# fdeguire03/InteriorPoint-GPU

Hardware: AMD Instinct MI355X
Metric: Newton iters/sec, dense QP n=8192, 1/2/4/8 GPUs; achieved % fp64 roofline (higher is better)
Workload: dtype f64

## Files before the change

### interiorpoint-gpu_amd/csrc/ipm_blas.hip

```cpp
#include <atomic>
#include "ipm_common.h"
#include <cstdio>
#include "ipm_mfma.h"

#include <algorithm>
#include <map>
#include <mutex>
#include <queue>
#include <cmath>
#include <tuple>
#include <vector>
#include <cstdlib>
#include <cstring>

namespace ipm {

static inline int64_t cdiv(int64_t a, int64_t b) { return (a + b - 1) / b; }

template <bool VEC>
__device__ __forceinline__ void gemv_row(int64_t row, int64_t cols, double alpha, const double* __restrict__ M,
                                         int64_t ldm, const double* __restrict__ x, double beta,
                                         double* __restrict__ y) {
  const int lane = threadIdx.x & 63;
  const double* mr = M + row * ldm;
// ... 1197 lines not shown
      if (16 * jt >= next_nb) break;
      const int64_t col0 = k0 + nb + 16 * jt;
      dbl4 acc;
#pragma unroll
      for (int r = 0; r < 4; ++r)
        acc[r] = (rfold && 16 * jt + fk + 4 * r < next_nb)
                     ? (FUSED ? ld_sc1(&A[(col0 + fk + 4 * r) * lda + row]) : A[(col0 + fk + 4 * r) * lda + row])
                     : 0.0;
      const double* sb = stage + jl * SLAB + fk * 16 + fr;
#pragma unroll
      for (int P = 0; P < 8; ++P)
#pragma unroll
        for (int s4 = 0; s4 < 4; ++s4)
          acc = __builtin_amdgcn_mfma_f64_16x16x4f64(-sb[(16 * P + 4 * s4) * 16], x[P][s4], acc, 0, 0, 0);
      if (rfold) {
#pragma unroll
        for (int r = 0; r < 4; ++r)
          if (16 * jt + fk + 4 * r < next_nb) {
            if (FUSED) st_sc1(&A[(col0 + fk + 4 * r) * lda + row], acc[r]);
            else A[(col0 + fk + 4 * r) * lda + row] = acc[r];
          }
      }
    }
  }
  }
  }
  if (done) {
    asm volatile("s_waitcnt vmcnt(0)" ::: "memory");
    __syncthreads();
    if (tid == 0) __hip_atomic_store(done, 1u, __ATOMIC_RELAXED, __HIP_MEMORY_SCOPE_AGENT);
  }
}

struct BlockArgs {
  int64_t n = 0, lda = 0;
  double* A = nullptr;
  int* info = nullptr;
  double* wsA = nullptr;
  double* wsB = nullptr;
  unsigned* ctl = nullptr;
  const unsigned* prevfail = nullptr;
  int64_t cb = 0;
  int wa = 0, wbw = 0;
  int nla = 0, nra = 0, nrb = 0, la_tj = 0, nlab = 0;
  int64_t ns = 0;
  int nnf = 0;
  GemmArgs la32, la, la128, s;
  int nla32 = 0, la32_T = 0, nla64 = 0, nla128 = 0;
  int trace = 0;
  int64_t rag_r0 = 0;
  int rag_n = 0, nrag = 0;
  int64_t s_full = 0;
  double* sscr = nullptr;
  unsigned* sflag = nullptr;
  int64_t nstrip = 0, f0 = 0;
  GemmArgs s2;
  int rag_K = CH_NB;
  int64_t rag_cp = 0;
  int ntail = 0, tail_r = 0, tail_R = 0, tail_K = 0;
  int64_t tail_o = 0, tail_k0 = 0;
};
__device__ __forceinline__ unsigned cu_key() {
  const unsigned hw = __builtin_amdgcn_s_getreg((31 << 11) | 4);
  const unsigned xcc = __builtin_amdgcn_s_getreg((31 << 11) | 20);
  return ((xcc & 15u) << 8) | ((hw >> 8) & 0xFFu);
}
// ... 12 lines not shown
  __syncthreads();
}

#ifdef IPM_ROLE_TRACE
__device__ unsigned long long ipm_role_trace[8192 * 4];
struct RoleTrace {
  bool on;
  int ticket;
  unsigned long long t0;
  int role = -1;
  unsigned long long wake = 0, loaded = 0;
  __device__ RoleTrace(bool o, int t) : on(o && t < 8192), ticket(t), t0(__builtin_amdgcn_s_memrealtime()) {}
  __device__ ~RoleTrace() {
    if (on && threadIdx.x == 0) {
      const unsigned lo = wake ? (unsigned)(loaded - t0) : (unsigned)ticket;
      ipm_role_trace[4 * ticket] = (unsigned long long)lo | ((unsigned long long)(unsigned)role << 32);
      ipm_role_trace[4 * ticket + 1] = t0;
      ipm_role_trace[4 * ticket + 2] = __builtin_amdgcn_s_memrealtime();
      ipm_role_trace[4 * ticket + 3] = wake ? wake : cu_key();
    }
  }
};
#define ROLE(r) (rt.role = (r))
#define ROLE_STAMP(f) (rt.f = __builtin_amdgcn_s_memrealtime())
__device__ unsigned long long ipm_fold_trace[32 * 12];
#define FOLD_SLOT ((frole == 0 ? 0 : 16) + ftile)
#define FOLD_STAMP(i) do { if (rt.on && ftile < 16 && tid == 0) ipm_fold_trace[FOLD_SLOT * 12 + (i)] = __builtin_amdgcn_s_memrealtime(); } while (0)
#else
#define FOLD_STAMP(i) do {} while (0)
#define ROLE(r) ((void)0)
#define ROLE_STAMP(f) ((void)0)
#endif

template <bool VEC, bool FASTS, int LAZY>
__device__ __forceinline__ void potrf_block_body(const BlockArgs& b, int64_t t, BlockSmem& sm, int& sflag) {
  const int tid = threadIdx.x;
  unsigned* const failw = &b.ctl[CTL_FAIL];
#ifdef IPM_ROLE_TRACE
  RoleTrace rt(b.trace != 0, (int)t);
#endif
  const int64_t t_launch = t;
  auto prev_failed = [&]() {
    const unsigned pf = ld_ctl(const_cast<unsigned*>(b.prevfail));
    if (pf == 0) return false;
    if (t_launch == 0 && tid == 0) __hip_atomic_store(&b.ctl[CTL_FAIL], pf, __ATOMIC_RELAXED, __HIP_MEMORY_SCOPE_AGENT);
    return true;
  };
  if (!(VEC && t < b.nla32 && (b.la32.K % 128) == 0) && prev_failed()) return;
  unsigned* la_done = b.ctl + CTL_HDR;
  unsigned* pa_done = la_done + (b.n + 63) / 64;
  int64_t fo = 0, fsrc = 0;
  int fni = 0, fnj = 0, fnp = 0;
  int ftile = 0, frole = 9;
  unsigned* fdone = nullptr;
  bool fwait = false;
  const bool la_fold = VEC && t < b.nla32 && (b.la32.K % 128) == 0;
  if (t < b.nla && !la_fold) {
    ROLE(0);
    int64_t rb;
    if (t < b.nla32) {
      mfma_tile<32, false, VEC, 2, true>(b.la32, t, sm.g32);
      int64_t i = (int64_t)((sqrt(8.0 * (double)t + 1.0) - 1.0) * 0.5);
      while ((i + 1) * (i + 2) / 2 <= t) ++i;
      while (i * (i + 1) / 2 > t) --i;
      rb = i >> 1;
    } else if (t - b.nla32 < b.nla64) {
      const int64_t t64 = t - b.nla32;
// ... 251 lines not shown
      const bool live = p < R * r && j <= i;
      double acc = 0.0;
      if (live)
        for (int k = q; k < K; k += 16) acc = fma(Ls[i * K + k], Ls[j * K + k], acc);
#pragma unroll
      for (int m = 8; m >= 1; m >>= 1) acc += __shfl_xor(acc, m, 16);
      if (live && q == 0) Cs[i * r + j] = ld_sc1(&b.A[(o + j) * lda + o + i]) - acc;
    }
    __syncthreads();
    int fcol = 0;
    for (int j = 0; j < r; ++j) {
      if (tid >= j && tid < R) {
        double v = Cs[tid * r + j];
        for (int k = 0; k < j; ++k) v = fma(-Cs[tid * r + k], Cs[j * r + k], v);
        Ts[tid] = v;
      }
      __syncthreads();
      const double piv = Ts[j], dv = rsqrt_pivot(piv);
      if (!(piv > 0.0) && fcol == 0) fcol = j + 1;
      if (tid >= j && tid < R) Cs[tid * r + j] = tid == j ? piv * dv : Ts[tid] * dv;
      __syncthreads();
    }
    if (tid < R)
      for (int j = 0; j < r && j <= tid; ++j) b.A[(o + j) * lda + o + tid] = Cs[tid * r + j];
    if (fcol && tid == 0) {
      atomicCAS(b.info, 0, (int)(o + fcol));
      __hip_atomic_store(failw, (unsigned)(o + fcol), __ATOMIC_RELAXED, __HIP_MEMORY_SCOPE_AGENT);
    }
    return;
  }
  if (kind == K_RAG) {
    ROLE(12);
    const int64_t o = b.cb + b.wa + b.wbw, cp = b.rag_cp;
    const int64_t m = b.n - o, r0 = b.rag_r0;
    const int rn = b.rag_n, KR = b.rag_K;
    double* xr = sm.d.sD;
    for (int e = tid; e < rn * KR; e += 256) {
      const int q = e / KR, k = e - q * KR;
      xr[e] = b.A[(cp + k) * b.lda + o + r0 + q];
    }
    __syncthreads();
    const int64_t j = t * 256 + tid;
    if (j < m) {
      double* cj = b.A + (o + j) * b.lda + o + r0;
      double acc[8];
#pragma unroll
      for (int q = 0; q < 8; ++q) acc[q] = (q < rn && j <= r0 + q) ? cj[q] : 0.0;
      const double* xp = b.A + cp * b.lda + o + j;
#pragma unroll 16
      for (int k = 0; k < KR; ++k) {
        const double xj = xp[k * b.lda];
#pragma unroll
        for (int q = 0; q < 8; ++q)
          if (q < rn) acc[q] = fma(-xj, xr[q * KR + k], acc[q]);
      }
#pragma unroll
      for (int q = 0; q < 8; ++q)
        if (q < rn && j <= r0 + q) cj[q] = acc[q];
    }
    return;
  }
  if (kind == K_TILE) {
    ROLE(4);
    {
        const int64_t st0 = t;
        const bool strip = st0 < b.nstrip;
        const int64_t st = strip ? st0 : st0 - b.nstrip, u = strip ? -1 : st - b.s_full;
        const int sp = u < 0 ? 0 : ((u & 1) ? 2 : 1);
        const int64_t p = u < 0 ? 0 : (u >> 1);
        GemmArgs g = b.s;
        if (strip) {
          g.ni = b.s2.ni;
          g.nj = b.s2.nj;
          g.X = b.s2.X;
          g.Y = b.s2.Y;
          g.C = b.s2.C;
          g.rowmajor = 1;
          g.xcd_remap = 0;
          g.tiles_i = b.s2.tiles_i;
          g.tiles_j = b.s2.tiles_j;
          g.nblk = b.s2.nblk;
        }
        mfma_tile<128, false, VEC, 2, false, false, (FASTS && VEC) ? 1 : 0, (FASTS && VEC) ? LAZY : 0>(
            g, strip ? st + (st >= 1 ? 1 : 0)
                     : b.f0 + (u < 0 ? st : b.s_full + p),
            sm.g128, sp, b.sscr + p * (128 * 128), b.sflag + p, -1, -1, b.info, failw);
    }
  }
}

template <bool VEC, bool FASTS = false, int LAZY = 0>
__global__ __launch_bounds__(256, 2) void k_potrf_block(BlockArgs b_arg) {
  IPM_KARGS(BlockArgs, b, b_arg);
  __shared__ BlockSmem sm;
  __shared__ int sticket, sflag;
  if (threadIdx.x == 0) sticket = (int)atomicAdd(&b.ctl[CTL_TICKET], 1u);
  __syncthreads();
  potrf_block_body<VEC, FASTS, LAZY>(b, __builtin_amdgcn_readfirstlane(sticket), sm, sflag);
}

static constexpr int64_t PANEL_WS = PF_DINV + 36 * 256;

__global__ void k_zero2(unsigned* a, int64_t na, unsigned* b, int64_t nb) {
  const int64_t i = (int64_t)blockIdx.x * 256 + threadIdx.x;
  if (i < na) a[i] = 0u;
  else if (i - na < nb) b[i - na] = 0u;
}
__global__ void k_zero2_border(unsigned* a, int64_t na, unsigned* b, int64_t nb, BorderJob j) {
  const int64_t i = (int64_t)blockIdx.x * 256 + threadIdx.x;
  if (i < na) a[i] = 0u;
  else if (i - na < nb) b[i - na] = 0u;
  else {
    const int64_t c = i - na - nb;
    if (c < j.N) j.H[c * j.ldh + j.N] = j.scale * j.g[c];
    else if (c == j.N) j.H[j.N * j.ldh + j.N] = j.corner;
  }
}
static void zero2(hipStream_t st, void* a, int64_t na, void* b, int64_t nb) {
  const int64_t tot = na + nb;
  if (tot > 0)
    hipLaunchKernelGGL(k_zero2, dim3((unsigned)cdiv(tot, 256)), dim3(256), 0, st, reinterpret_cast<unsigned*>(a), na,
                       reinterpret_cast<unsigned*>(b), nb);
}

static int num_cus();
static double split_makespan(int slots, const std::vector<std::pair<int64_t, double>>& items) {
  std::priority_queue<double, std::vector<double>, std::greater<double>> q;
  for (int i = 0; i < slots; ++i) q.push(0.0);
  double mk = 0.0;
  for (const auto& it : items)
    for (int64_t k = 0; k < it.first; ++k) {
      const double t = q.top() + it.second;
      q.pop();
      q.push(t);
      mk = std::max(mk, t);
    }
  return mk;
}
static std::vector<std::pair<int64_t, double>> launch_items(int64_t nla, int64_t nchd, int64_t nnf, bool pb,
                                                            int64_t nrag, int64_t nstrip, int64_t ns, int64_t q,
                                                            double tc, double lac, int64_t nra, int64_t nrb,
                                                            int64_t sa, int64_t sb) {
  std::vector<std::pair<int64_t, double>> it = {{nla, lac}, {1, 0.6}, {nchd, 0.66}, {nnf, 0.8}, {pb ? 1 : 0, 1.25},
                                                {nrag, 0.1 * tc}};
  const int64_t e1 = nstrip + ns - q, e2 = e1 + 2 * q;
  auto span = [&](int64_t a, int64_t z) {
    const int64_t w1 = std::max<int64_t>(0, std::min(z, e1) - a);
    const int64_t w2 = std::max<int64_t>(0, std::min(z, e2) - std::max(a, e1));
    if (w1 > 0) it.push_back({w1, tc});
    if (w2 > 0) it.push_back({w2, 0.55 * tc});
  };
  sa = std::min(sa, e2);
  sb = std::min(std::max(sb, sa), e2);
  span(0, sa);
  it.push_back({nra, 0.5});
  span(sa, sb);
  it.push_back({nrb, 0.5});
  span(sb, e2);
  return it;
}
static int64_t plan_split(int64_t nla, int64_t nchd, int64_t nnf, bool pb, int64_t nrag, int64_t ns, int64_t nrows,
                          int64_t cap, double tc = 1.0, int64_t nstrip = 0, double lac = 0.8, int64_t nra = -1,
                          int64_t sa = -1, int64_t sb = -1) {
  if (ns < 64) return 0;
  const int slots = 2 * num_cus();
  if (nra < 0) {
    nra = nrows;
    sa = sb = nstrip + ns;
  }
  const int64_t nrb = nrows - nra;
  auto mk = [&](int64_t q) {
    int64_t a = sa, z = sb;
    return split_makespan(slots, launch_items(nla, nchd, nnf, pb, nrag, nstrip, ns, q, tc, lac, nra, nrb, a, z));
  };
  const double m0 = mk(0);
  double best = m0;
  int64_t bq = 0;
  for (int64_t q = 8; q <= std::min(ns, cap); q += 8) {
    const double m = mk(q);
    if (m < best - 0.02) { best = m; bq = q; }
  }
  return bq;
}

struct PairPlan {
  std::vector<int> kind;
  std::vector<int64_t> f1;
};
static PairPlan potrf_pair_plan(int64_t n, int64_t ncols, int64_t nblocks) {
  PairPlan pl;
  pl.kind.assign(nblocks, 0);
  pl.f1.assign(nblocks, 0);
  static const bool on = [] { const char* e = getenv("IPM_PAIR"); return !(e && e[0] == '0'); }();
  static const int64_t minrows = [] { const char* e = getenv("IPM_PAIR_MIN"); return e ? atoll(e) : 6144LL; }();
  if (!on || ncols < n - 8) return pl;
  int64_t last = -1;
  for (int64_t e = 2; e + 1 < nblocks; e += 2) {
    if (n - (e + 2) * CH_NB < minrows) break;
    last = e;
  }
  if (last < 0) return pl;
  pl.kind[1] = 1;
  for (int64_t e = 2; e <= last; e += 2) {
    pl.kind[e] = 2;
    if (e < last) pl.kind[e + 1] = 1;
  }
  return pl;
}

static unsigned long long wall_ticks(unsigned us) {
  static long long khz = -1;
  if (khz < 0) {
    int dev = 0, v = 0;
    hipGetDevice(&dev);
    khz = (hipDeviceGetAttribute(&v, hipDeviceAttributeWallClockRate, dev) == hipSuccess && v > 0) ? v : 100000;
  }
  const unsigned long long t = (unsigned long long)us * (unsigned long long)khz / 1000ull;
  return t > 0 ? t : 1;
}
constexpr unsigned SPIN_US_DEFAULT = 1000000;
static void set_spin_ticks(int which, unsigned us) {
  const unsigned long long t = wall_ticks(us ? us : SPIN_US_DEFAULT);
  int cur = 0, cnt = 0;
  hipGetDevice(&cur);
  if (hipGetDeviceCount(&cnt) != hipSuccess || cnt < 1) cnt = 1;
  for (int d = 0; d < cnt; ++d) {
    if (hipSetDevice(d) != hipSuccess) continue;
    hipMemcpyToSymbol(HIP_SYMBOL(ipm_spin_ticks), &t, sizeof(t), which * sizeof(t), hipMemcpyHostToDevice);
  }
  hipSetDevice(cur);
}
void set_potrf_spin_limit_us(unsigned us) { set_spin_ticks(0, us); }

struct BlockLaunch {
  BlockArgs b;
  int64_t grid = 0;
  int inst = 4;
};
static void potrf_plan(int64_t n, double* A, int64_t lda, int* info, double* ws, int64_t ncols,
                       std::vector<BlockLaunch>& out) {
  out.clear();
  const int64_t nblocks = cdiv(ncols, CH_NB), cw = block_ctl_words(n);
  unsigned* ctl0 = reinterpret_cast<unsigned*>(ws + 2 * PANEL_WS);
  const bool vec = ((lda & 1) == 0) && ((((uintptr_t)A) & 15) == 0);
  const char* erag = getenv("IPM_RAG");
  const bool rag_on = erag ? erag[0] != '0' : n > 5120;
  const char* esp = getenv("IPM_SPLIT");
  const bool split_on = !(esp && esp[0] == '0');
  const char* elz = getenv("IPM_LAZYC");
  const bool lazy_on = !(elz && elz[0] == '0');
  const bool lazy2_on = lazy_on && !(elz && elz[0] == '1');
  PairPlan pl = potrf_pair_plan(n, ncols, nblocks);
  const char* etl = getenv("IPM_TAIL");
  const bool tail_on = !(etl && etl[0] == '0');
  int64_t nemit = nblocks;
  int tail_r = 0;
  if (tail_on && nblocks >= 2 && pl.kind[nblocks - 2] == 0) {
    const int64_t cbl = (nblocks - 1) * CH_NB;
    if (ncols - cbl <= 8 && n - cbl <= 16) {
      nemit = nblocks - 1;
      tail_r = (int)(ncols - cbl);
    }
  }
  for (int64_t bk = 0; bk < nemit; ++bk) {
    const int kind = pl.kind[bk];
    const int64_t Kla = kind == 2 ? 2 * CH_NB : CH_NB;
    BlockArgs b;
    b.n = n;
    b.lda = lda;
    b.A = A;
    b.info = info;
    b.wsA = ws;
    b.wsB = ws + PANEL_WS;
    b.ctl = ctl0 + 8 + bk * cw;
    b.prevfail = bk == 0 ? ctl0 : ctl0 + 8 + (bk - 1) * cw + CTL_FAIL;
    const int64_t cb = bk * CH_NB, wb = std::min<int64_t>(CH_NB, ncols - cb);
    b.cb = cb;
    b.wa = (int)std::min<int64_t>(wb, PF_NB);
    b.wbw = (int)(wb - b.wa);
    if (bk > 0) {
      const int64_t cp = cb - Kla;
      const int64_t ni = n - cb;
      GemmArgs& c = b.la32;
      c.ni = std::min<int64_t>(ni, 128);
// ... 44 lines not shown
      b.nla = b.nla32 + b.nla64 + b.nla128;
      b.la_tj = (int)a.tiles_j;
      b.nlab = (int)cdiv(ni, 64);
      const int64_t m = n - cb - wb;
      b.rag_cp = cb - CH_NB;
      b.rag_K = CH_NB;
      if (m > 0 && kind == 1) {
        if (bk >= 1 && pl.kind[bk - 1] == 2) {
          const int64_t me = m + CH_NB;
          const int64_t rn = (rag_on && me > 128 && (me & 127) != 0 && (me & 127) <= 8) ? (me & 127) : 0;
          const int64_t mF = m - rn;
          GemmArgs& g = b.s;
          g.ni = g.nj = mF;
          g.K = 2 * CH_NB;
          g.X = g.Y = A + (cb - 3 * CH_NB) * lda + cb + wb;
          g.ldx = g.ldy = lda;
          g.C = A + (cb + wb) * lda + cb + wb;
          g.ldc = lda;
          g.sub = 1;
          g.tri = 1;
          g.xcd_remap = 1;
          g.tiles_i = cdiv(mF, 128);
          g.nblk = g.tiles_i * (g.tiles_i + 1) / 2;
          b.f0 = pl.f1[bk - 1];
          b.s_full = g.nblk - b.f0;
          b.ns = b.s_full;
        }
      } else if (m > 0 && kind == 2) {
        int64_t ms = m;
        if (rag_on && m > 128 && (m & 127) != 0 && (m & 127) <= 8) {
          ms = m - (m & 127);
          b.rag_r0 = ms;
          b.rag_n = (int)(m & 127);
          b.nrag = (int)cdiv(m, 256);
          b.rag_cp = cp;
          b.rag_K = (int)Kla;
        }
        const int64_t o = cb + wb, mF = ms - CH_NB;
        GemmArgs& s2 = b.s2;
        s2.ni = ms;
        s2.nj = CH_NB;
        s2.K = Kla;
        s2.X = s2.Y = A + cp * lda + o;
        s2.ldx = s2.ldy = lda;
        s2.C = A + o * lda + o;
        s2.ldc = lda;
        s2.sub = 1;
        s2.tri = 1;
        s2.rowmajor = 1;
        s2.xcd_remap = 0;
        s2.tiles_i = cdiv(ms, 128);
        s2.tiles_j = 2;
        s2.nblk = s2.tiles_i * 2;
        b.nstrip = s2.nblk - 1;
        GemmArgs& g = b.s;
        g = s2;
        g.rowmajor = 0;
        g.ni = g.nj = mF;
        g.X = g.Y = A + cp * lda + o + CH_NB;
        g.C = A + (o + CH_NB) * lda + o + CH_NB;
        g.xcd_remap = 1;
        g.tiles_i = cdiv(mF, 128);
        g.tiles_j = 0;
        g.nblk = g.tiles_i * (g.tiles_i + 1) / 2;
        const bool last = bk + 1 >= nblocks || pl.kind[bk + 1] != 1;
        const int64_t f1 = last ? g.nblk : std::max<int64_t>(0, std::min<int64_t>(g.nblk, (g.nblk - b.nstrip) / 2));
        pl.f1[bk] = f1;
        b.f0 = 0;
        b.s_full = f1;
        b.ns = b.nstrip + f1;
      } else if (m > 0) {
        GemmArgs& g = b.s;
        int64_t ms = m;
        if (rag_on && m > 128 && (m & 127) != 0 && (m & 127) <= 8) {
          ms = m - (m & 127);
          b.rag_r0 = ms;
          b.rag_n = (int)(m & 127);
          b.nrag = (int)cdiv(m, 256);
        }
        g.ni = g.nj = ms;
        g.K = CH_NB;
        g.X = g.Y = A + cp * lda + cb + wb;
        g.ldx = g.ldy = lda;
        g.C = A + (cb + wb) * lda + cb + wb;
        g.ldc = lda;
        g.sub = 1;
        g.tri = 1;
        g.xcd_remap = 1;
        g.tiles_i = cdiv(ms, 128);
        g.nblk = g.tiles_i * (g.tiles_i + 1) / 2;
        b.ns = g.nblk;
        b.s_full = b.ns;
      }
    }
    if (tail_r > 0 && bk == nemit - 1) {
      b.ns = b.s_full = b.nstrip = 0;
      b.nrag = 0;
      b.ntail = 1;
      b.tail_r = tail_r;
      b.tail_o = cb + CH_NB;
      b.tail_R = (int)(n - b.tail_o);
      b.tail_k0 = bk > 0 ? cb - CH_NB : 0;
      b.tail_K = (int)(b.tail_o - b.tail_k0);
    }
#ifdef IPM_ROLE_TRACE
    {
      static const int tb = [] { const char* e = getenv("IPM_TRACE_BLOCK"); return e ? atoi(e) : -1; }();
      b.trace = bk == tb;
    }
#endif
    b.nra = (int)cdiv(std::max<int64_t>(n - cb - b.wa, 0), PF_RB);
// ... 9 lines not shown
    if (b.s_full > 0 && split_here) {
      static std::mutex mu;
      static std::map<std::tuple<int64_t, int64_t, int>, std::vector<int64_t>> cache;
      const int nchd_h = b.wbw > 0 ? (b.wbw + PF_RB - 1) / PF_RB : 0;
      const double tc = b.s.K > CH_NB ? 1.6 : 1.0, lac = Kla > CH_NB ? 1.6 : 0.8;
      const int64_t nra_h = b.nra - nchd_h;
      int64_t q = 0;
      {
        std::lock_guard<std::mutex> lk(mu);
        auto& v = cache[{n, ncols, (lazy_on ? 4 : 0) | (lazy2_on ? 8 : 0) | (vec ? 16 : 0)}];
        if ((int64_t)v.size() < nblocks) v.assign(nblocks, -1);
        if (v[bk] < 0) {
          v[bk] = plan_split(b.nla, nchd_h, b.nnf, b.wbw > 0, b.nrag, b.s_full, nra_h + b.nrb, potrf_split_cap(n),
                             tc, b.nstrip, lac);
          static const bool dbg = getenv("IPM_SPLIT_DEBUG") != nullptr;
          if (dbg)
            fprintf(stderr, "potrf n=%ld block %ld: %ld trailing tiles, split %ld\n", (long)n, (long)bk, (long)b.ns,
                    (long)v[bk]);
        }
        q = v[bk];
      }
      b.s_full -= q;
      b.ns = b.nstrip + b.s_full + 2 * q;
      b.sscr = ws + potrf_split_scratch_off(n);
      b.sflag = b.ctl + block_ctl_words(n) - potrf_split_cap(n);
    }
    BlockLaunch L;
    L.grid = b.nla + 1 + b.nra + b.nnf + (b.wbw > 0 ? 1 + b.nrb : 0) + b.nrag + b.ns + b.ntail;
    const bool fasts = fasts_on && b.ns > 0 && (b.s.ni % 128) == 0 && (b.s.K % 32) == 0;
    const bool lazy = lazy_on && fasts && b.s.K == CH_NB && b.nstrip == 0 && b.s_full == b.ns;
    const bool lazy2 = lazy2_on && fasts && b.s.K == 2 * CH_NB && b.nstrip + b.s_full == b.ns &&
                       (b.nstrip == 0 || b.s2.K == 2 * CH_NB) && (b.nrag == 0 || b.rag_K <= 2 * CH_NB);
    L.inst = (vec && lazy) ? 0 : (vec && lazy2) ? 1 : (vec && fasts) ? 2 : vec ? 3 : 4;
    L.b = b;
    out.push_back(L);
  }
}

static void launch_block(hipStream_t st, const BlockLaunch& L) {
  const dim3 g((unsigned)L.grid), t(256);
  switch (L.inst) {
    case 0: hipLaunchKernelGGL((k_potrf_block<true, true, 1>), g, t, 0, st, L.b); break;
    case 1: hipLaunchKernelGGL((k_potrf_block<true, true, 2>), g, t, 0, st, L.b); break;
    case 2: hipLaunchKernelGGL((k_potrf_block<true, true>), g, t, 0, st, L.b); break;
    case 3: hipLaunchKernelGGL((k_potrf_block<true, false>), g, t, 0, st, L.b); break;
    default: hipLaunchKernelGGL((k_potrf_block<false, false>), g, t, 0, st, L.b); break;
  }
}

void potrf_lower_fused(hipStream_t st, int64_t n, double* A, int64_t lda, int* info, double* ws, int64_t ncols,
                       const BorderJob* border) {
  if (ncols < 0 || ncols > n) ncols = n;
  if (border && ncols <= 0) border_rhs(st, border->N, border->H, border->ldh, border->g, border->scale);
  if (ncols <= 0) {
    hipMemsetAsync(info, 0, sizeof(int), st);
    return;
  }
  thread_local std::vector<BlockLaunch> plan;
  potrf_plan(n, A, lda, info, ws, ncols, plan);
  unsigned* ctl0 = reinterpret_cast<unsigned*>(ws + 2 * PANEL_WS);
  if (border) {
    const int64_t nz = 8 + (int64_t)plan.size() * block_ctl_words(n), tot = 1 + nz + border->N + 1;
    hipLaunchKernelGGL(k_zero2_border, dim3((unsigned)cdiv(tot, 256)), dim3(256), 0, st, reinterpret_cast<unsigned*>(info),
                       (int64_t)1, ctl0, nz, *border);
  } else {
    zero2(st, info, 1, ctl0, 8 + (int64_t)plan.size() * block_ctl_words(n));
  }
  for (const BlockLaunch& L : plan) launch_block(st, L);
}

static int num_cus() {
  static int ncu = -1;
  if (ncu < 0) {
    int dev = 0, v = 0;
    hipGetDevice(&dev);
    ncu = (hipDeviceGetAttribute(&v, hipDeviceAttributeMultiprocessorCount, dev) == hipSuccess && v > 0) ? v : 256;
  }
  return ncu;
// ... 831 lines not shown
```

### interiorpoint-gpu_amd/csrc/ipm_mfma.h

```cpp
#pragma once
#include <algorithm>
#include <map>
#include <mutex>
#include <queue>
#include <tuple>
#include <type_traits>
#include <vector>

#include "ipm_common.h"

namespace ipm {

#ifdef IPM_TILE_STAMPS
__device__ unsigned long long ipm_tile_stamps[4096 * 8];
#define IPM_TSTAMP(k) do { if (threadIdx.x == 0 && blockIdx.x < 4096) ipm_tile_stamps[blockIdx.x * 8 + (k)] = __builtin_amdgcn_s_memtime(); } while (0)
#define IPM_TSTAMPR(k) do { if (threadIdx.x == 0 && blockIdx.x < 4096) ipm_tile_stamps[blockIdx.x * 8 + (k)] = __builtin_amdgcn_s_memrealtime(); } while (0)
#else
#define IPM_TSTAMP(k) do {} while (0)
#define IPM_TSTAMPR(k) do {} while (0)
#endif

struct GemmArgs {
  int64_t ni = 0, nj = 0, K = 0;
  const double* X = nullptr;
// ... 26 lines not shown
      reinterpret_cast<unsigned long long*>(const_cast<double*>(p)), __ATOMIC_RELAXED, __HIP_MEMORY_SCOPE_AGENT));
}
__device__ __forceinline__ void st_sc1(double* p, double v) {
  __hip_atomic_store(reinterpret_cast<unsigned long long*>(p), (unsigned long long)__double_as_longlong(v),
                     __ATOMIC_RELAXED, __HIP_MEMORY_SCOPE_AGENT);
}

static __device__ unsigned long long ipm_spin_ticks[2] = {100000000ull, 100000000ull};
__device__ __forceinline__ void spin_fail(int* info, unsigned* failw) {
  if (info) atomicCAS(info, 0, POTRF_INFO_SPIN);
  __threadfence();
  if (failw) atomicCAS(failw, 0u, 0xFFFFFFF0u);
}
template <int SLEEP, int WHICH = 0, class Done>
__device__ __forceinline__ bool spin_until(int* info, unsigned* failw, Done done) {
  if (done()) return true;
  unsigned long long t0 = 0;
  for (unsigned it = 0;; ++it) {
    __builtin_amdgcn_s_sleep(SLEEP);
    if (done()) return true;
    if ((it & 15u) != 0u) continue;
    const unsigned long long now = __builtin_amdgcn_s_memrealtime();
    if (it == 0) {
      t0 = now;
      continue;
    }
    if (failw && __hip_atomic_load(failw, __ATOMIC_RELAXED, __HIP_MEMORY_SCOPE_AGENT) != 0u) return false;
    if (now - t0 > ipm_spin_ticks[WHICH]) {
      spin_fail(info, failw);
      return false;
    }
  }
}

template <int BM_, int WJ = 2>
struct MfCfg {
  static constexpr int BM = BM_, BK = 16, NT = 128 * WJ;
  static constexpr int LD = BM + 16;
  static constexpr int PT = BK * BM / NT;
  static constexpr int TPR = BM / PT;
  static constexpr int TWI = BM / 32;
  static constexpr int TWJ = BM / (16 * WJ);
};

template <int BM_, int WJ = 2>
struct alignas(16) MfSmem {
  alignas(16) double sX[2][MfCfg<BM_, WJ>::BK * MfCfg<BM_, WJ>::LD];
  alignas(16) double sY[2][MfCfg<BM_, WJ>::BK * MfCfg<BM_, WJ>::LD];
};

template <int BM_, bool WEIGHT, bool VEC, int WJ = 2, bool SC1OUT = false, bool SPLITADD = false, int LOOP = 0,
          int LAZYC = 0, bool CST = false>
__device__ __forceinline__ void mfma_tile(const GemmArgs& a, int64_t Lw, MfSmem<BM_, WJ>& sm, int SPLIT = 0,
                                          double* part = nullptr, unsigned* pflag = nullptr, int64_t kb = -1,
                                          int64_t ke = -1, int* sinfo = nullptr, unsigned* failw = nullptr) {
  using M = MfCfg<BM_, WJ>;
  constexpr int BM = M::BM, BK = M::BK, LD = M::LD, PT = M::PT, TPR = M::TPR, TWI = M::TWI, TWJ = M::TWJ;
  IPM_TSTAMP(0);
  IPM_TSTAMPR(6);
#ifdef IPM_TILE_STAMPS
  if (threadIdx.x == 0 && blockIdx.x < 4096)
    ipm_tile_stamps[blockIdx.x * 8 + 5] = ((unsigned long long)__builtin_amdgcn_s_getreg((31 << 11) | 20) << 32) |
                                          __builtin_amdgcn_s_getreg((31 << 11) | 4);
#endif
  auto& sX = sm.sX;
  auto& sY = sm.sY;
// ... 51 lines not shown
          ry[2 * q + 1] = v.y;
        }
      } else {
#pragma unroll
        for (int q = 0; q < PT; ++q) {
          rx[q] = (WEIGHT ? xs[q] * wk : xs[q]) * xsg;
          ry[q] = ys[q];
        }
      }
    } else {
      const bool kin = k < Kt;
      const double wk = (WEIGHT && kin) ? a.w[kbeg + k] : 1.0;
#pragma unroll
      for (int q = 0; q < PT; ++q) {
        const bool xi = kin && (I0 + sc + q < a.ni), yj = kin && (J0 + sc + q < a.nj);
        rx[q] = xi ? (WEIGHT ? xs[q] * wk : xs[q]) * xsg : 0.0;
        ry[q] = yj ? ys[q] : 0.0;
      }
    }
  };
  auto sstore = [&](int buf) {
#pragma unroll
    for (int q = 0; q < PT; ++q) {
      sX[buf][sr * LD + sc + q] = rx[q];
      sY[buf][sr * LD + sc + q] = ry[q];
    }
  };
  const int fr = lane & 15, fk = lane >> 4;
  dbl4 acc[TWJ][TWI];
#pragma unroll
  for (int u = 0; u < TWJ; ++u)
#pragma unroll
    for (int v = 0; v < TWI; ++v) acc[u][v] = dbl4{0.0, 0.0, 0.0, 0.0};
  static_assert(!LAZYC || (LOOP == 1 && !WEIGHT), "lazy C: fast loop, no weight");
  static_assert(!CST || (LOOP == 1 && !LAZYC && BM_ == 128 && WJ == 2), "staged C: 128-tile fast loop");
  constexpr int CLD = 144;
  double* sCst = &sm.sX[0][0];
  static_assert(!CST || 4 * BK * LD >= 64 * CLD, "staging fits the slab buffers");
  if (CST && cinit && SPLIT == 0) {
#pragma unroll
    for (int h = 0; h < 2; ++h) {
#pragma unroll
      for (int q = 0; q < 16; ++q) {
        const int e = tid + 256 * q, col = e >> 6, rp = e & 63;
        const double2 v = *reinterpret_cast<const double2*>(a.C + (J0 + 64 * h + col) * a.ldc + I0 + 2 * rp);
        *reinterpret_cast<double2*>(&sCst[col * CLD + 2 * rp]) = v;
      }
      __syncthreads();
      if (wj == h) {
#pragma unroll
        for (int tj = 0; tj < TWJ; ++tj)
#pragma unroll
          for (int ti = 0; ti < TWI; ++ti)
#pragma unroll
            for (int r = 0; r < 4; ++r)
              acc[tj][ti][r] = sCst[(tj * 16 + fk + 4 * r) * CLD + wi * (BM / 2) + ti * 16 + fr];
      }
      __syncthreads();
    }
  } else if (cinit && SPLIT != 1 && !LAZYC) {
#pragma unroll
    for (int tj = 0; tj < TWJ; ++tj)
#pragma unroll
      for (int ti = 0; ti < TWI; ++ti) {
        const int64_t i = I0 + wi * (BM / 2) + ti * 16 + fr;
#pragma unroll
        for (int r = 0; r < 4; ++r) {
          const int64_t j = J0 + wj * (BM / WJ) + tj * 16 + fk + 4 * r;
          acc[tj][ti][r] = (i < a.ni && j < a.nj) ? (SC1OUT ? ld_sc1(&a.C[j * a.ldc + i]) : a.C[j * a.ldc + i]) : 0.0;
        }
      }
  }
  static_assert(LOOP == 0 || (BM_ == 128 && VEC && WJ == 2), "fast loop: 128-tiles, vector loads");
  if constexpr (LAZYC) {
    double fx[PT], fy[PT];
    auto fload = [&](int64_t s) {
      const double2* xs = reinterpret_cast<const double2*>(xp + s * xstep);
      const double2* ys = reinterpret_cast<const double2*>(yp + s * ystep);
#pragma unroll
      for (int q = 0; q < PT / 2; ++q) {
        const double2 u = xs[q], v = ys[q];
        fx[2 * q] = u.x;
        fx[2 * q + 1] = u.y;
        fy[2 * q] = v.x;
        fy[2 * q + 1] = v.y;
      }
    };
    auto fstore = [&](int buf) {
#pragma unroll
      for (int q = 0; q < PT; ++q) {
        sX[buf][sr * LD + sc + q] = fx[q] * xsg;
        sY[buf][sr * LD + sc + q] = fy[q];
      }
    };
    auto cload = [&](int q) {
      const int tj = q / TWI, ti = q % TWI;
      const int64_t i = I0 + wi * (BM / 2) + ti * 16 + fr;
      const int64_t j0 = J0 + wj * (BM / WJ) + tj * 16 + fk;
      dbl4 v;
#pragma unroll
      for (int r = 0; r < 4; ++r) v[r] = a.C[(j0 + 4 * r) * a.ldc + i];
      return v;
    };
    constexpr int NS = 16, R = LAZYC > 0 ? LAZYC : 1, NSL = NS * R;
    static_assert(TWJ * TWI == NS, "one accumulator block per R slabs");
    dbl4 cq[NS];
    fload(0);
    fstore(0);
    fload(1);
    cq[0] = cload(0);
    __syncthreads();
#pragma unroll
    for (int s = 0; s < NSL; ++s) {
      const int buf = s & 1;
      const double* bx = sX[buf];
      const double* by = sY[buf];
      fstore(buf ^ 1);
      fload(s + 2 < NSL ? s + 2 : NSL - 1);
      if (s % R == 0) {
        const int q = s / R;
        if (q + 1 < NS) cq[q + 1] = cload(q + 1);
        if (q >= 2) acc[(q - 2) / TWI][(q - 2) % TWI] += cq[q - 2];
      }
      __builtin_amdgcn_sched_barrier(0);
#pragma unroll
      for (int kk = 0; kk < BK / 4; ++kk) {
        double av[TWJ], bv[TWI];
#pragma unroll
        for (int t = 0; t < TWJ; ++t) av[t] = by[(kk * 4 + fk) * LD + wj * (BM / WJ) + t * 16 + fr];
#pragma unroll
        for (int t = 0; t < TWI; ++t) bv[t] = bx[(kk * 4 + fk) * LD + wi * (BM / 2) + t * 16 + fr];
#pragma unroll
        for (int tj = 0; tj < TWJ; ++tj)
#pragma unroll
          for (int ti = 0; ti < TWI; ++ti)
            acc[tj][ti] = __builtin_amdgcn_mfma_f64_16x16x4f64(av[tj], bv[ti], acc[tj][ti], 0, 0, 0);
      }
      __syncthreads();
    }
    acc[(NS - 2) / TWI][(NS - 2) % TWI] += cq[NS - 2];
    acc[(NS - 1) / TWI][(NS - 1) % TWI] += cq[NS - 1];
  } else if (LOOP == 1) {
    double fx[PT], fy[PT];
    double fw = 1.0;
    auto fload = [&](int64_t s) {
      const double2* xs = reinterpret_cast<const double2*>(xp + s * xstep);
      const double2* ys = reinterpret_cast<const double2*>(yp + s * ystep);
#pragma unroll
      for (int q = 0; q < PT / 2; ++q) {
        const double2 u = xs[q], v = ys[q];
        fx[2 * q] = u.x;
        fx[2 * q + 1] = u.y;
        fy[2 * q] = v.x;
        fy[2 * q + 1] = v.y;
      }
      if (WEIGHT) fw = a.w[kbeg + s * BK + sr];
    };
    auto fstore = [&](int buf) {
#pragma unroll
      for (int q = 0; q < PT; ++q) {
        sX[buf][sr * LD + sc + q] = (WEIGHT ? fx[q] * fw : fx[q]) * xsg;
        sY[buf][sr * LD + sc + q] = fy[q];
      }
    };
    fload(0);
    fstore(0);
    fload(nslab > 1 ? 1 : 0);
    __syncthreads();
    IPM_TSTAMP(1);
    for (int64_t s = 0; s < nslab; ++s) {
      const int buf = (int)(s & 1);
// ... 142 lines not shown
      spin_until<2>(sinfo, failw, [&] { return __hip_atomic_load(pflag, __ATOMIC_RELAXED, __HIP_MEMORY_SCOPE_AGENT) != 0u; });
    __syncthreads();
  }
  if (CST && cinit && SPLIT == 0) {
    const bool diag = a.tri && I0 == J0;
#pragma unroll
    for (int h = 0; h < 2; ++h) {
      if (wj == h) {
#pragma unroll
        for (int tj = 0; tj < TWJ; ++tj)
#pragma unroll
          for (int ti = 0; ti < TWI; ++ti)
#pragma unroll
            for (int r = 0; r < 4; ++r)
              sCst[(tj * 16 + fk + 4 * r) * CLD + wi * (BM / 2) + ti * 16 + fr] = acc[tj][ti][r];
      }
      __syncthreads();
#pragma unroll
      for (int q = 0; q < 16; ++q) {
        const int e = tid + 256 * q, col = e >> 6, rp = e & 63;
        const double2 v = *reinterpret_cast<const double2*>(&sCst[col * CLD + 2 * rp]);
        double* cp = a.C + (J0 + 64 * h + col) * a.ldc + I0 + 2 * rp;
        const int c = 64 * h + col;
        if (!diag || 2 * rp >= c) {
          *reinterpret_cast<double2*>(cp) = v;
        } else if (2 * rp + 1 == c) {
          cp[1] = v.y;
        }
      }
      if (h == 0) __syncthreads();
    }
    return;
  }
  constexpr bool PRE = LOOP >= 2;
#pragma unroll
  for (int tj = 0; tj < TWJ; ++tj) {
    double pp[TWI][4], pc[TWI][4];
    if constexpr (PRE) {
      if (!cinit && SPLIT != 1) {
#pragma unroll
        for (int ti = 0; ti < TWI; ++ti) {
          const int64_t i = I0 + wi * (BM / 2) + ti * 16 + fr;
#pragma unroll
          for (int r = 0; r < 4; ++r) {
            const int64_t j = J0 + wj * (BM / WJ) + tj * 16 + fk + 4 * r;
            const bool ok = i < a.ni && j < a.nj && (!a.tri || i >= j);
            pp[ti][r] = (ok && a.P) ? a.P[j * a.ldp + i] : 0.0;
            pc[ti][r] = (ok && a.beta != 0.0) ? a.C[j * a.ldc + i] : 0.0;
          }
        }
      }
    }
#pragma unroll
    for (int ti = 0; ti < TWI; ++ti) {
      const int64_t i = I0 + wi * (BM / 2) + ti * 16 + fr;
#pragma unroll
      for (int r = 0; r < 4; ++r) {
        const int64_t j = J0 + wj * (BM / WJ) + tj * 16 + fk + 4 * r;
        if (SPLIT == 1) {
          st_sc1(&part[(j - J0) * BM + (i - I0)], acc[tj][ti][r]);
        } else if (i < a.ni && j < a.nj && (!a.tri || i >= j)) {
          double* cp = a.C + j * a.ldc + i;
          if (cinit) {
            double v = acc[tj][ti][r];
            if (SPLIT == 2) v += ld_sc1(&part[(j - J0) * BM + (i - I0)]);
            if (SC1OUT) st_sc1(cp, v);
            else *cp = v;
// ... 365 lines not shown
```

Measured before the change: 121.7.

## Split ragged-row update K across waves with vector loads; add opt-in register-ring trailing loop

Rewrites the ragged-row Cholesky update so each workgroup covers 128 columns, splits the K reduction across four waves with double2 loads and an LDS partial-sum reduction, and retunes its cost in the split scheduler. This is meant to raise parallelism and memory throughput for the ragged tail, which previously used one thread per column over the whole K. It also adds an optional trailing-tile loop variant that streams the X operand from global memory into a register ring instead of staging it in LDS, selected by an environment variable and off by default. The trade-off is more workgroups and an extra LDS reduction and barrier per workgroup.

```diff
diff --git a/interiorpoint-gpu_amd/csrc/ipm_blas.hip b/interiorpoint-gpu_amd/csrc/ipm_blas.hip
--- a/interiorpoint-gpu_amd/csrc/ipm_blas.hip
+++ b/interiorpoint-gpu_amd/csrc/ipm_blas.hip
@@ -1253,6 +1253,9 @@
   }
 }
 
+constexpr int RAG_W = 128;
+static_assert(CH_NB % 128 == 0 && 2 * CH_NB <= 512,
+              "ragged rows: each wave's quarter of K is whole batches of 32, 8 staged rows of a pair's K fit their LDS");
 struct BlockArgs {
   int64_t n = 0, lda = 0;
   double* A = nullptr;
@@ -1331,7 +1334,7 @@
 #define ROLE_STAMP(f) ((void)0)
 #endif
 
-template <bool VEC, bool FASTS, int LAZY>
+template <bool VEC, bool FASTS, int LAZY, int SLOOP>
 __device__ __forceinline__ void potrf_block_body(const BlockArgs& b, int64_t t, BlockSmem& sm, int& sflag) {
   const int tid = threadIdx.x;
   unsigned* const failw = &b.ctl[CTL_FAIL];
@@ -1649,32 +1652,86 @@
   if (kind == K_RAG) {
     ROLE(12);
     const int64_t o = b.cb + b.wa + b.wbw, cp = b.rag_cp;
-    const int64_t m = b.n - o, r0 = b.rag_r0;
+    const int64_t m = b.n - o, r0 = b.rag_r0, lda = b.lda;
     const int rn = b.rag_n, KR = b.rag_K;
-    double* xr = sm.d.sD;
-    for (int e = tid; e < rn * KR; e += 256) {
-      const int q = e / KR, k = e - q * KR;
-      xr[e] = b.A[(cp + k) * b.lda + o + r0 + q];
-    }
-    __syncthreads();
-    const int64_t j = t * 256 + tid;
-    if (j < m) {
-      double* cj = b.A + (o + j) * b.lda + o + r0;
-      double acc[8];
-#pragma unroll
-      for (int q = 0; q < 8; ++q) acc[q] = (q < rn && j <= r0 + q) ? cj[q] : 0.0;
-      const double* xp = b.A + cp * b.lda + o + j;
-#pragma unroll 16
-      for (int k = 0; k < KR; ++k) {
-        const double xj = xp[k * b.lda];
-#pragma unroll
-        for (int q = 0; q < 8; ++q)
-          if (q < rn) acc[q] = fma(-xj, xr[q * KR + k], acc[q]);
-      }
-#pragma unroll
-      for (int q = 0; q < 8; ++q)
-        if (q < rn && j <= r0 + q) cj[q] = acc[q];
-    }
+    const int lane = tid & 63, wv = tid >> 6;
+    const int64_t j0 = t * RAG_W;
+    auto rag = [&](auto nrc, auto vecc) {
+      constexpr int NR = decltype(nrc)::value;
+      constexpr bool V = decltype(vecc)::value;
+      constexpr int NE = NR * RAG_W / 256;
+      double* xr = sm.d.sD;
+      double* part = xr + 8 * 512;
+      static_assert(8 * 512 + 4 * 8 * RAG_W <= 36 * 256, "ragged rows: staged rows + partials fit sD");
+      for (int e = tid; e < NR * KR; e += 256) {
+        const int k = e / NR, q = e - k * NR;
+        const double v = b.A[(cp + k) * lda + o + r0 + std::min(q, rn - 1)];
+        xr[e] = q < rn ? v : 0.0;
+      }
+      double cv[NE];
+      double* cptr[NE];
+      bool ok[NE];
+#pragma unroll
+      for (int i = 0; i < NE; ++i) {
+        const int e = tid + 256 * i, q = e / RAG_W;
+        const int64_t j = j0 + (e % RAG_W);
+        ok[i] = q < rn && j < m && j <= r0 + q;
+        cptr[i] = b.A + (o + std::min(j, m - 1)) * lda + o + r0 + std::min(q, rn - 1);
+        cv[i] = *cptr[i];
+      }
+      __syncthreads();
+      const int KQ = KR >> 2, kq0 = wv * KQ;
+      const int64_t jl = j0 + 2 * lane, ja = std::min(jl, m - 1), jb = std::min(jl + 1, m - 1);
+      const double* xp = b.A + (cp + kq0) * lda + o;
+      double a0[NR], a1[NR];
+#pragma unroll
+      for (int q = 0; q < NR; ++q) a0[q] = a1[q] = 0.0;
+      for (int k0 = 0; k0 < KQ; k0 += 32) {
+        double2 v[32];
+#pragma unroll
+        for (int u = 0; u < 32; ++u) {
+          const double* p = xp + (int64_t)(k0 + u) * lda;
+          if constexpr (V) {
+            v[u] = *reinterpret_cast<const double2*>(p + jl);
+          } else {
+            v[u].x = p[ja];
+            v[u].y = p[jb];
+          }
+        }
+#pragma unroll
+        for (int u = 0; u < 32; ++u) {
+          const double* xk = xr + (kq0 + k0 + u) * NR;
+#pragma unroll
+          for (int q = 0; q < NR; ++q) {
+            a0[q] = fma(v[u].x, xk[q], a0[q]);
+            a1[q] = fma(v[u].y, xk[q], a1[q]);
+          }
+        }
+      }
+#pragma unroll
+      for (int q = 0; q < NR; ++q)
+        *reinterpret_cast<double2*>(&part[(wv * NR + q) * RAG_W + 2 * lane]) = double2{a0[q], a1[q]};
+      __syncthreads();
+#pragma unroll
+      for (int i = 0; i < NE; ++i) {
+        const int e = tid + 256 * i;
+        double s = part[e] + part[NR * RAG_W + e];
+        s += part[2 * NR * RAG_W + e];
+        s += part[3 * NR * RAG_W + e];
+        if (ok[i]) *cptr[i] = cv[i] - s;
+      }
+    };
+    using std::integral_constant;
+    const bool vrag = VEC && (o & 1) == 0 && j0 + RAG_W <= m;
+    if constexpr (VEC) {
+      if (vrag) {
+        if (rn <= 2) rag(integral_constant<int, 2>{}, std::true_type{});
+        else rag(integral_constant<int, 8>{}, std::true_type{});
+        return;
+      }
+    }
+    if (rn <= 2) rag(integral_constant<int, 2>{}, std::false_type{});
+    else rag(integral_constant<int, 8>{}, std::false_type{});
     return;
   }
   if (kind == K_TILE) {
@@ -1698,7 +1755,7 @@
           g.tiles_j = b.s2.tiles_j;
           g.nblk = b.s2.nblk;
         }
-        mfma_tile<128, false, VEC, 2, false, false, (FASTS && VEC) ? 1 : 0, (FASTS && VEC) ? LAZY : 0>(
+        mfma_tile<128, false, VEC, 2, false, false, (FASTS && VEC) ? (LAZY ? SLOOP : 1) : 0, (FASTS && VEC) ? LAZY : 0>(
             g, strip ? st + (st >= 1 ? 1 : 0)
                      : b.f0 + (u < 0 ? st : b.s_full + p),
             sm.g128, sp, b.sscr + p * (128 * 128), b.sflag + p, -1, -1, b.info, failw);
@@ -1706,14 +1763,14 @@
   }
 }
 
-template <bool VEC, bool FASTS = false, int LAZY = 0>
+template <bool VEC, bool FASTS = false, int LAZY = 0, int SLOOP = 1>
 __global__ __launch_bounds__(256, 2) void k_potrf_block(BlockArgs b_arg) {
   IPM_KARGS(BlockArgs, b, b_arg);
   __shared__ BlockSmem sm;
   __shared__ int sticket, sflag;
   if (threadIdx.x == 0) sticket = (int)atomicAdd(&b.ctl[CTL_TICKET], 1u);
   __syncthreads();
-  potrf_block_body<VEC, FASTS, LAZY>(b, __builtin_amdgcn_readfirstlane(sticket), sm, sflag);
+  potrf_block_body<VEC, FASTS, LAZY, SLOOP>(b, __builtin_amdgcn_readfirstlane(sticket), sm, sflag);
 }
 
 static constexpr int64_t PANEL_WS = PF_DINV + 36 * 256;
@@ -1759,7 +1816,7 @@
                                                             double tc, double lac, int64_t nra, int64_t nrb,
                                                             int64_t sa, int64_t sb) {
   std::vector<std::pair<int64_t, double>> it = {{nla, lac}, {1, 0.6}, {nchd, 0.66}, {nnf, 0.8}, {pb ? 1 : 0, 1.25},
-                                                {nrag, 0.1 * tc}};
+                                                {nrag, 0.04 * tc}};
   const int64_t e1 = nstrip + ns - q, e2 = e1 + 2 * q;
   auto span = [&](int64_t a, int64_t z) {
     const int64_t w1 = std::max<int64_t>(0, std::min(z, e1) - a);
@@ -1808,8 +1865,10 @@
   PairPlan pl;
   pl.kind.assign(nblocks, 0);
   pl.f1.assign(nblocks, 0);
-  static const bool on = [] { const char* e = getenv("IPM_PAIR"); return !(e && e[0] == '0'); }();
-  static const int64_t minrows = [] { const char* e = getenv("IPM_PAIR_MIN"); return e ? atoll(e) : 6144LL; }();
+  const char* epr = getenv("IPM_PAIR");
+  const bool on = !(epr && epr[0] == '0');
+  const char* epm = getenv("IPM_PAIR_MIN");
+  const int64_t minrows = epm ? atoll(epm) : 6144LL;
   if (!on || ncols < n - 8) return pl;
   int64_t last = -1;
   for (int64_t e = 2; e + 1 < nblocks; e += 2) {
@@ -1849,6 +1908,7 @@
 }
 void set_potrf_spin_limit_us(unsigned us) { set_spin_ticks(0, us); }
 
+constexpr int STILE_LOOP_DEFAULT = 1;
 struct BlockLaunch {
   BlockArgs b;
   int64_t grid = 0;
@@ -1867,6 +1927,8 @@
   const char* elz = getenv("IPM_LAZYC");
   const bool lazy_on = !(elz && elz[0] == '0');
   const bool lazy2_on = lazy_on && !(elz && elz[0] == '1');
+  const char* esl = getenv("IPM_STILE_LOOP");
+  const int stile_loop = esl ? (esl[0] == '1' ? 1 : 2) : STILE_LOOP_DEFAULT;
   PairPlan pl = potrf_pair_plan(n, ncols, nblocks);
   const char* etl = getenv("IPM_TAIL");
   const bool tail_on = !(etl && etl[0] == '0');
@@ -1977,7 +2039,7 @@
           ms = m - (m & 127);
           b.rag_r0 = ms;
           b.rag_n = (int)(m & 127);
-          b.nrag = (int)cdiv(m, 256);
+          b.nrag = (int)cdiv(m, RAG_W);
           b.rag_cp = cp;
           b.rag_K = (int)Kla;
         }
@@ -2021,7 +2083,7 @@
           ms = m - (m & 127);
           b.rag_r0 = ms;
           b.rag_n = (int)(m & 127);
-          b.nrag = (int)cdiv(m, 256);
+          b.nrag = (int)cdiv(m, RAG_W);
         }
         g.ni = g.nj = ms;
         g.K = CH_NB;
@@ -2097,6 +2159,13 @@
     const bool lazy2 = lazy2_on && fasts && b.s.K == 2 * CH_NB && b.nstrip + b.s_full == b.ns &&
                        (b.nstrip == 0 || b.s2.K == 2 * CH_NB) && (b.nrag == 0 || b.rag_K <= 2 * CH_NB);
     L.inst = (vec && lazy) ? 0 : (vec && lazy2) ? 1 : (vec && fasts) ? 2 : vec ? 3 : 4;
+    if (L.inst <= 1 && stile_loop == 2) L.inst += 5;
+    {
+      static const bool dbg = getenv("IPM_PLAN_DEBUG") != nullptr;
+      if (dbg)
+        fprintf(stderr, "potrf n=%ld block %ld: kernel %d, %ld trailing tiles (K = %ld), %d ragged-row workgroups (K = %d)\n",
+                (long)n, (long)bk, L.inst, (long)b.ns, (long)b.s.K, b.nrag, b.rag_K);
+    }
     L.b = b;
     out.push_back(L);
   }
@@ -2109,6 +2178,8 @@
     case 1: hipLaunchKernelGGL((k_potrf_block<true, true, 2>), g, t, 0, st, L.b); break;
     case 2: hipLaunchKernelGGL((k_potrf_block<true, true>), g, t, 0, st, L.b); break;
     case 3: hipLaunchKernelGGL((k_potrf_block<true, false>), g, t, 0, st, L.b); break;
+    case 5: hipLaunchKernelGGL((k_potrf_block<true, true, 1, 2>), g, t, 0, st, L.b); break;
+    case 6: hipLaunchKernelGGL((k_potrf_block<true, true, 2, 2>), g, t, 0, st, L.b); break;
     default: hipLaunchKernelGGL((k_potrf_block<false, false>), g, t, 0, st, L.b); break;
   }
 }
diff --git a/interiorpoint-gpu_amd/csrc/ipm_mfma.h b/interiorpoint-gpu_amd/csrc/ipm_mfma.h
--- a/interiorpoint-gpu_amd/csrc/ipm_mfma.h
+++ b/interiorpoint-gpu_amd/csrc/ipm_mfma.h
@@ -82,6 +82,10 @@
     }
   }
 }
+
+#ifndef IPM_STILE_XRING
+#define IPM_STILE_XRING 3
+#endif
 
 template <int BM_, int WJ = 2>
 struct MfCfg {
@@ -199,7 +203,7 @@
   for (int u = 0; u < TWJ; ++u)
 #pragma unroll
     for (int v = 0; v < TWI; ++v) acc[u][v] = dbl4{0.0, 0.0, 0.0, 0.0};
-  static_assert(!LAZYC || (LOOP == 1 && !WEIGHT), "lazy C: fast loop, no weight");
+  static_assert(!LAZYC || ((LOOP == 1 || LOOP == 2) && !WEIGHT), "lazy C: a fast loop, no weight");
   static_assert(!CST || (LOOP == 1 && !LAZYC && BM_ == 128 && WJ == 2), "staged C: 128-tile fast loop");
   constexpr int CLD = 144;
   double* sCst = &sm.sX[0][0];
@@ -240,26 +244,6 @@
   }
   static_assert(LOOP == 0 || (BM_ == 128 && VEC && WJ == 2), "fast loop: 128-tiles, vector loads");
   if constexpr (LAZYC) {
-    double fx[PT], fy[PT];
-    auto fload = [&](int64_t s) {
-      const double2* xs = reinterpret_cast<const double2*>(xp + s * xstep);
-      const double2* ys = reinterpret_cast<const double2*>(yp + s * ystep);
-#pragma unroll
-      for (int q = 0; q < PT / 2; ++q) {
-        const double2 u = xs[q], v = ys[q];
-        fx[2 * q] = u.x;
-        fx[2 * q + 1] = u.y;
-        fy[2 * q] = v.x;
-        fy[2 * q + 1] = v.y;
-      }
-    };
-    auto fstore = [&](int buf) {
-#pragma unroll
-      for (int q = 0; q < PT; ++q) {
-        sX[buf][sr * LD + sc + q] = fx[q] * xsg;
-        sY[buf][sr * LD + sc + q] = fy[q];
-      }
-    };
     auto cload = [&](int q) {
       const int tj = q / TWI, ti = q % TWI;
       const int64_t i = I0 + wi * (BM / 2) + ti * 16 + fr;
@@ -272,38 +256,119 @@
     constexpr int NS = 16, R = LAZYC > 0 ? LAZYC : 1, NSL = NS * R;
     static_assert(TWJ * TWI == NS, "one accumulator block per R slabs");
     dbl4 cq[NS];
-    fload(0);
-    fstore(0);
-    fload(1);
-    cq[0] = cload(0);
-    __syncthreads();
-#pragma unroll
-    for (int s = 0; s < NSL; ++s) {
-      const int buf = s & 1;
-      const double* bx = sX[buf];
-      const double* by = sY[buf];
-      fstore(buf ^ 1);
-      fload(s + 2 < NSL ? s + 2 : NSL - 1);
-      if (s % R == 0) {
-        const int q = s / R;
-        if (q + 1 < NS) cq[q + 1] = cload(q + 1);
-        if (q >= 2) acc[(q - 2) / TWI][(q - 2) % TWI] += cq[q - 2];
-      }
-      __builtin_amdgcn_sched_barrier(0);
-#pragma unroll
-      for (int kk = 0; kk < BK / 4; ++kk) {
-        double av[TWJ], bv[TWI];
-#pragma unroll
-        for (int t = 0; t < TWJ; ++t) av[t] = by[(kk * 4 + fk) * LD + wj * (BM / WJ) + t * 16 + fr];
-#pragma unroll
-        for (int t = 0; t < TWI; ++t) bv[t] = bx[(kk * 4 + fk) * LD + wi * (BM / 2) + t * 16 + fr];
-#pragma unroll
-        for (int tj = 0; tj < TWJ; ++tj)
-#pragma unroll
-          for (int ti = 0; ti < TWI; ++ti)
-            acc[tj][ti] = __builtin_amdgcn_mfma_f64_16x16x4f64(av[tj], bv[ti], acc[tj][ti], 0, 0, 0);
-      }
+    if constexpr (LOOP == 2) {
+      double fy[PT];
+      auto fload = [&](int64_t s) {
+        const double2* ys = reinterpret_cast<const double2*>(yp + s * ystep);
+#pragma unroll
+        for (int q = 0; q < PT / 2; ++q) {
+          const double2 v = ys[q];
+          fy[2 * q] = v.x;
+          fy[2 * q + 1] = v.y;
+        }
+      };
+      auto fstore = [&](int buf) {
+#pragma unroll
+        for (int q = 0; q < PT; ++q) sY[buf][sr * LD + sc + q] = fy[q];
+      };
+      const double* xq = a.X + (kbeg + fk) * a.ldx + I0 + wi * (BM / 2) + fr;
+      constexpr int XRING = IPM_STILE_XRING, G = NSL * (BK / 4);
+      double xr[XRING][TWI];
+      auto xload = [&](int g) {
+        const double* p = xq + (int64_t)(g * 4) * a.ldx;
+#pragma unroll
+        for (int t = 0; t < TWI; ++t) xr[g % XRING][t] = p[t * 16] * xsg;
+      };
+      fload(0);
+      fstore(0);
+      fload(1);
+#pragma unroll
+      for (int g = 0; g < XRING; ++g) xload(g);
+      cq[0] = cload(0);
       __syncthreads();
+#pragma unroll
+      for (int s = 0; s < NSL; ++s) {
+        const int buf = s & 1;
+        const double* by = sY[buf];
+        fstore(buf ^ 1);
+        fload(s + 2 < NSL ? s + 2 : NSL - 1);
+        if (s % R == 0) {
+          const int q = s / R;
+          if (q + 1 < NS) cq[q + 1] = cload(q + 1);
+          if (q >= 2) acc[(q - 2) / TWI][(q - 2) % TWI] += cq[q - 2];
+        }
+        __builtin_amdgcn_sched_barrier(0);
+#pragma unroll
+        for (int kk = 0; kk < BK / 4; ++kk) {
+          const int g = s * (BK / 4) + kk;
+          double av[TWJ], bv[TWI];
+#pragma unroll
+          for (int t = 0; t < TWJ; ++t) av[t] = by[(kk * 4 + fk) * LD + wj * (BM / WJ) + t * 16 + fr];
+#pragma unroll
+          for (int t = 0; t < TWI; ++t) bv[t] = xr[g % XRING][t];
+          if (g + XRING < G) xload(g + XRING);
+#pragma unroll
+          for (int tj = 0; tj < TWJ; ++tj)
+#pragma unroll
+            for (int ti = 0; ti < TWI; ++ti)
+              acc[tj][ti] = __builtin_amdgcn_mfma_f64_16x16x4f64(av[tj], bv[ti], acc[tj][ti], 0, 0, 0);
+        }
+        __syncthreads();
+      }
+    } else {
+      double fx[PT], fy[PT];
+      auto fload = [&](int64_t s) {
+        const double2* xs = reinterpret_cast<const double2*>(xp + s * xstep);
+        const double2* ys = reinterpret_cast<const double2*>(yp + s * ystep);
+#pragma unroll
+        for (int q = 0; q < PT / 2; ++q) {
+          const double2 u = xs[q], v = ys[q];
+          fx[2 * q] = u.x;
+          fx[2 * q + 1] = u.y;
+          fy[2 * q] = v.x;
+          fy[2 * q + 1] = v.y;
+        }
+      };
+      auto fstore = [&](int buf) {
+#pragma unroll
+        for (int q = 0; q < PT; ++q) {
+          sX[buf][sr * LD + sc + q] = fx[q] * xsg;
+          sY[buf][sr * LD + sc + q] = fy[q];
+        }
+      };
+      fload(0);
+      fstore(0);
+      fload(1);
+      cq[0] = cload(0);
+      __syncthreads();
+#pragma unroll
+      for (int s = 0; s < NSL; ++s) {
+        const int buf = s & 1;
+        const double* bx = sX[buf];
+        const double* by = sY[buf];
+        fstore(buf ^ 1);
+        fload(s + 2 < NSL ? s + 2 : NSL - 1);
+        if (s % R == 0) {
+          const int q = s / R;
+          if (q + 1 < NS) cq[q + 1] = cload(q + 1);
+          if (q >= 2) acc[(q - 2) / TWI][(q - 2) % TWI] += cq[q - 2];
+        }
+        __builtin_amdgcn_sched_barrier(0);
+#pragma unroll
+        for (int kk = 0; kk < BK / 4; ++kk) {
+          double av[TWJ], bv[TWI];
+#pragma unroll
+          for (int t = 0; t < TWJ; ++t) av[t] = by[(kk * 4 + fk) * LD + wj * (BM / WJ) + t * 16 + fr];
+#pragma unroll
+          for (int t = 0; t < TWI; ++t) bv[t] = bx[(kk * 4 + fk) * LD + wi * (BM / 2) + t * 16 + fr];
+#pragma unroll
+          for (int tj = 0; tj < TWJ; ++tj)
+#pragma unroll
+            for (int ti = 0; ti < TWI; ++ti)
+              acc[tj][ti] = __builtin_amdgcn_mfma_f64_16x16x4f64(av[tj], bv[ti], acc[tj][ti], 0, 0, 0);
+        }
+        __syncthreads();
+      }
     }
     acc[(NS - 2) / TWI][(NS - 2) % TWI] += cq[NS - 2];
     acc[(NS - 1) / TWI][(NS - 1) % TWI] += cq[NS - 1];
@@ -512,7 +577,7 @@
     }
     return;
   }
-  constexpr bool PRE = LOOP >= 2;
+  constexpr bool PRE = LOOP >= 2 && !LAZYC;
 #pragma unroll
   for (int tj = 0; tj < TWJ; ++tj) {
     double pp[TWI][4], pc[TWI][4];
```

Measured after the change: 123.7, median of 6. 1.6% higher.
